# PixArt-alpha/PixArt-sigma

Hardware: AMD Instinct MI355X
Metric: denoising steps/sec (fwd+bwd) PixArt-Sigma-XL/2 1024px bs16 @1/2/4/8 GPU (higher is better)
Workload: dtype fp16; 1 GPU; PixArt-Sigma-XL/2 1024px training step (fwd+bwd+clip+AdamW), batch 16/GPU, L=300 text tokens, DP=1 RCCL all-reduce; model=PixArtMS_XL_2, global_batch=16, seq_len=4096, parallelism=dp1, grad_checkpoint=False, optimizer=adamw, text_lens=all 300

## Files before the change

### pixart_sigma_amd/csrc/attn.hip

```cpp
#include "common.h"
#include "../../include/pixart_hip.h"
#include <utility>
#include <cstdlib>

namespace {
using namespace pxa;

constexpr int DH = 72;
constexpr int NCH = DH / 8;
constexpr int KSTEPS = 5;
constexpr int ROWB = 192;
constexpr int TILE_B = 64 * ROWB;
constexpr int BKV = 64;
constexpr float RESCALE_LOG2 = 6.0f;
constexpr int NDMA = TILE_B / 1024 / 4;

struct AttnParams {
  const bf16_t *Q, *K, *V, *dO;
  bf16_t *O, *dQ, *dK, *dV;
  float* LSE;
  const float* Delta;
  float *dq_colsum, *dk_colsum, *dv_colsum;
  long colsum_stride;
  long q_bs, q_ts, k_bs, k_ts, v_bs, v_ts, o_bs, o_ts;
  int q_hs, k_hs, v_hs, o_hs;
  long dq_bs, dq_ts, dk_bs, dk_ts, dv_bs, dv_ts;
  int dq_hs, dk_hs, dv_hs;
  int B, H, Nq, Nk;
  const int* kv_start; const int* kv_len;
  float scale, scale_log2;
  float dk_scale;
  int nx;
  const bf16_t* stats;
  int Nq64;
};

#ifndef ATTN_XCD_HEADS
#define ATTN_XCD_HEADS 1
#endif
__device__ __forceinline__ void block_coords(const AttnParams& p, int& bx, int& h, int& b) {
  int v = blockIdx.x;
#if ATTN_XCD_HEADS
  const int T = gridDim.x, xq = T >> 3, xr = T & 7, xcd = v & 7;
  v = xcd * xq + min(xcd, xr) + (v >> 3);
#endif
  bx = v % p.nx;
  const int hb = v / p.nx;
  h = hb % p.H;
  b = hb / p.H;
}

__device__ __forceinline__ void kv_range(const AttnParams& p, int b, long& kbase, long& vbase, long& dkbase, long& dvbase, int& len) {
  if (p.kv_start) {
    const long s = p.kv_start[b];
    kbase = s * p.k_ts; vbase = s * p.v_ts; dkbase = s * p.dk_ts; dvbase = s * p.dv_ts; len = p.kv_len[b];
  } else {
    kbase = (long)b * p.k_bs; vbase = (long)b * p.v_bs; dkbase = (long)b * p.dk_bs; dvbase = (long)b * p.dv_bs; len = p.Nk;
  }
}


__device__ __forceinline__ int soff(int r, int c) { return r * ROWB + ((c ^ ((r >> 2) & 3)) << 4); }

__device__ __forceinline__ void tile_sync() {
  lds_dma_wait<0>();
  __syncthreads();
}
__device__ __forceinline__ void settle(bf16x8 (&f)[5]) { asm volatile("" : "+v"(f[0]), "+v"(f[1]), "+v"(f[2]), "+v"(f[3]), "+v"(f[4])); }
struct DmaPlan { int row[NDMA], coff[NDMA]; };
__device__ __forceinline__ void dma_plan(DmaPlan& pl, int wave, int lane) {
#pragma unroll
  for (int i = 0; i < NDMA; i++) {
    const int p = (i * 4 + wave) * 64 + lane, r = p / 12, cl = p - r * 12;
    const int c = cl ^ ((r >> 2) & 3);
    pl.row[i] = r;
    pl.coff[i] = c < NCH ? c * 8 : -1;
  }
}
template <bool FULL>
__device__ __forceinline__ void dma_tile(char* lds, const bf16_t* __restrict__ base, int ts, int row0, int nrows, const DmaPlan& pl, int wave) {
#pragma unroll
  for (int i = 0; i < NDMA; i++) {
    const int gr = FULL ? row0 + pl.row[i] : min(row0 + pl.row[i], nrows - 1);
    const unsigned off = (unsigned)(gr * ts + pl.coff[i]);
    if (pl.coff[i] >= 0)
      lds_dma16(base + off, lds + (i * 4 + wave) * 1024);
  }
}
#ifndef ATTN_FOLD_DELTA
#define ATTN_FOLD_DELTA 1
#endif
#define PXA_OPERAND_MINUS_ONE_X2 (((PXA_OPERAND_ONE_BITS | 0x8000u) << 16) | PXA_OPERAND_ONE_BITS | 0x8000u)
#define PXA_OPERAND_MINUS_ONE_X1 (PXA_OPERAND_ONE_BITS | 0x8000u)
__device__ __forceinline__ uint2 split3(float x) {
  const bf16_t h = (bf16_t)x;
  const float r1 = x - (float)h;
  const bf16_t m = (bf16_t)r1;
  const bf16_t l = (bf16_t)(r1 - (float)m);
  bf16x2 a, b; a[0] = h; a[1] = m; b[0] = l; b[1] = (bf16_t)0.f;
  return make_uint2(__builtin_bit_cast(uint32_t, a), __builtin_bit_cast(uint32_t, b));
}
__device__ __forceinline__ void init_pads(char* tile, int pad, int tid) {
  for (int i = tid; i < BKV * 3; i += 256) {
// ... 1551 lines not shown
    if (j + 1 >= T) break;
    body(IntC<1>{});
    kdma += j + 7 < T ? kstep : 0;  vdma += j + 5 < T ? vstep : 0;
    if (j + 2 >= T) break;
    body(IntC<2>{});
    kdma += j + 8 < T ? kstep : 0;  vdma += j + 6 < T ? vstep : 0;
    if (j + 3 >= T) break;
    body(IntC<3>{});
    kdma += j + 9 < T ? kstep : 0;  vdma += j + 7 < T ? vstep : 0;
  }
  lds_wait_all<0>(kf);
  lds_dma_wait<0>();
#if FWD4_TRACE
  if (blockIdx.x == 0 && tid == 0) { fwd4_trace_buf[0] = tr_wait; fwd4_trace_buf[1] = tr_a; fwd4_trace_buf[2] = tr_b; fwd4_trace_buf[3] = tr_n; }
#endif

  mfma_drain();
#pragma unroll
  for (int s = 0; s < QS; s++) {
    const float la = __shfl(o[s].v[4][0][0], 32 + (lane & 15)), lb = __shfl(o[s].v[4][1][0], 32 + (lane & 15));
    const float l = (lane & 16) ? lb : la;
    const float inv = l > 0.f ? 1.f / l : 0.f, invo = __shfl_xor(inv, 16);
    const int q0w = bx * 256 + wave * 64 + s * 32;
    store_rows16(p.O + (long)b * p.o_bs + (long)q0w * p.o_ts + (long)h * p.o_hs, p.o_ts, o[s], (lane & 16) ? invo : inv, (lane & 16) ? inv : invo,
                 q0w + (lane & 15) < p.Nq, q0w + 16 + (lane & 15) < p.Nq, lane);
    if (qvalid[s] && hi == 0 && p.LSE) p.LSE[((long)b * p.H + h) * p.Nq + q[s]] = mc[s] + log2f(l);
  }
}

#define PXA_WAIT_STR "s_waitcnt lgkmcnt(%3)\n\t"
template <int W = -1> __device__ __forceinline__ void mfma32_va_first(f32x16& d, const bf16x8& a, const bf16x8& b) {
  if constexpr (W >= 0) asm volatile(PXA_WAIT_STR PXA_MFMA32_ASM " %0, %1, %2, 0" : "=&v"(d) : "v"(a), "a"(b), "n"(W));
  else asm volatile(PXA_MFMA32_ASM " %0, %1, %2, 0" : "=&v"(d) : "v"(a), "a"(b));
}
template <int W = -1> __device__ __forceinline__ void mfma32_va(f32x16& d, const bf16x8& a, const bf16x8& b) {
  if constexpr (W >= 0) asm volatile(PXA_WAIT_STR PXA_MFMA32_ASM " %0, %1, %2, %0" : "+v"(d) : "v"(a), "a"(b), "n"(W));
  else asm volatile(PXA_MFMA32_ASM " %0, %1, %2, %0" : "+v"(d) : "v"(a), "a"(b));
}
template <int W = -1> __device__ __forceinline__ void mfma32_vv_first(f32x16& d, const bf16x8& a, const bf16x8& b) {
  if constexpr (W >= 0) asm volatile(PXA_WAIT_STR PXA_MFMA32_ASM " %0, %1, %2, 0" : "=&v"(d) : "v"(a), "v"(b), "n"(W));
  else asm volatile(PXA_MFMA32_ASM " %0, %1, %2, 0" : "=&v"(d) : "v"(a), "v"(b));
}
template <int W = -1> __device__ __forceinline__ void mfma32_vv(f32x16& d, const bf16x8& a, const bf16x8& b) {
  if constexpr (W >= 0) asm volatile(PXA_WAIT_STR PXA_MFMA32_ASM " %0, %1, %2, %0" : "+v"(d) : "v"(a), "v"(b), "n"(W));
  else asm volatile(PXA_MFMA32_ASM " %0, %1, %2, %0" : "+v"(d) : "v"(a), "v"(b));
}
template <int W = -1> __device__ __forceinline__ void mfma32_acc(f32x16& d, const bf16x8& a, const bf16x8& b) {
  if constexpr (W >= 0) asm volatile(PXA_WAIT_STR PXA_MFMA32_ASM " %0, %1, %2, %0" : "+a"(d) : "v"(a), "v"(b), "n"(W));
  else asm volatile(PXA_MFMA32_ASM " %0, %1, %2, %0" : "+a"(d) : "v"(a), "v"(b));
}
#ifndef PXA_ATTN_DKV4_DEFAULT
#define PXA_ATTN_DKV4_DEFAULT 1
#endif
#ifndef DKV4_ABL
#define DKV4_ABL 0
#endif
constexpr int DKV4_STAGES = 4;
constexpr int dkv4_nreads(int i) { const int k = ((i % 22) + 22) % 22; return k < 10 ? 1 : 2; }
template <bool PRE>
__global__ __launch_bounds__(256, 1) void attn_bwd_dkv4_kernel(AttnParams p) {
  __shared__ __attribute__((aligned(16))) char smem[DKV4_STAGES * STAGE_B];
  const int tid = threadIdx.x, lane = tid & 63, wave = __builtin_amdgcn_readfirstlane(tid >> 6), hi = lane >> 5;
  int bx, h, b;
  block_coords(p, bx, h, b);
  const long kbase = (long)b * p.k_bs, vbase = (long)b * p.v_bs, dkbase = (long)b * p.dk_bs, dvbase = (long)b * p.dv_bs;
  typedef unsigned u32x4 __attribute__((ext_vector_type(4)));

  const bf16_t* Qp = p.Q + (long)b * p.q_bs + (long)h * p.q_hs;
  const bf16_t* Dp = p.dO + (long)b * p.o_bs + (long)h * p.o_hs;
  const bf16_t* Ls = p.stats + ((long)b * p.H + h) * p.Nq64 * 8;
  const bf16_t* Ds = Ls + (long)p.B * p.H * p.Nq64 * 8;
  const int qts = (int)p.q_ts, ots = (int)p.o_ts;
  const int T = p.Nq / BKV;
  const float c = p.scale_log2;

  DmaPlan pl;
  dma_plan(pl, wave, lane);
  unsigned offQ[NDMA], offD[NDMA];
  unsigned long long dmask[NDMA];
#pragma unroll
  for (int i = 0; i < NDMA; i++) {
    offQ[i] = (unsigned)(pl.row[i] * qts + pl.coff[i]) * 2u;
    offD[i] = (unsigned)(pl.row[i] * ots + pl.coff[i]) * 2u;
    dmask[i] = __builtin_amdgcn_ballot_w64(pl.coff[i] >= 0);
  }
  const unsigned lds0 = (unsigned)(uintptr_t)LDS_PTR(char, smem);
  const unsigned wbase = __builtin_amdgcn_readfirstlane(wave * 1024);
  const long qstep = (long)BKV * qts, ostep = (long)BKV * ots;
  const unsigned stat_off = (unsigned)lane * 16u;
  const bf16_t* statp = (wave & 1) ? Ds : Ls;
  const unsigned stat_dst = __builtin_amdgcn_readfirstlane((wave & 1) ? 2 * TILE_B + STAT_B : TILE_B);
  const bf16_t* qnext = Qp;
  const bf16_t* dnext = Dp;
  const bf16_t* snext = statp;
  auto issue_part = [&](auto pc, unsigned sb) {
    constexpr int P = decltype(pc)::value;
    const unsigned wb = wbase + sb, so = stat_off, sd = stat_dst + sb;
    const bf16_t* sn = snext;
    if constexpr (P == 0) dma_pair<0, TILE_B + STAT_B>(dmask[0], wb, offQ[0], qnext, offD[0], dnext);
    if constexpr (P == 1) dma_pair<4096, TILE_B + STAT_B + 4096>(dmask[1], wb, offQ[1], qnext, offD[1], dnext);
    if constexpr (P == 2) dma_pair<8192, TILE_B + STAT_B + 8192>(dmask[2], wb, offQ[2], qnext, offD[2], dnext);
    if constexpr (P == 3) asm volatile("s_mov_b32 m0, %0\n\ts_nop 0\n\tglobal_load_lds_dwordx4 %1, %2" :: "s"(sd), "v"(so), "s"(sn) : "memory");
  };
  int tfetch = 0;
  auto advance = [&]() {
    const bool more = tfetch + 1 < T;
    qnext += more ? qstep : 0; dnext += more ? ostep : 0; snext += more ? (long)BKV * 8 : 0;
    tfetch++;
  };
  auto issue = [&](unsigned sb) { issue_part(IntC<0>{}, sb); issue_part(IntC<1>{}, sb); issue_part(IntC<2>{}, sb); issue_part(IntC<3>{}, sb); advance(); };

  FragAddr fa;
  frag_addr(fa, lane);
  int r4[2];
#pragma unroll
  for (int sub = 0; sub < 2; sub++) r4[sub] = hi ? TILE_B + (sub * 32 + (lane & 31)) * 16 : fa.rb[0] + 2 * 64 + sub * 32 * ROWB;
  struct Bases { unsigned r0, r1, r40, r41, t0, t1; };
  auto bases = [&](unsigned st) -> Bases { return Bases{st + (unsigned)fa.rb[0], st + (unsigned)fa.rb[1], st + (unsigned)r4[0], st + (unsigned)r4[1],
                                                        st + (unsigned)fa.tb[0], st + (unsigned)fa.tb[1]}; };
  constexpr int DOFF = TILE_B + STAT_B;

  for (int st = 0; st < DKV4_STAGES; st++) {
    init_pads(smem + st * STAGE_B, 0, tid);
    init_pads(smem + st * STAGE_B + DOFF, 0, tid);
  }
  f32x16 dk[2][3], dv[2][3];
#pragma unroll
  for (int kb = 0; kb < 2; kb++) {
    zero3(dk[kb]); zero3(dv[kb]);
#pragma unroll
    for (int dt = 0; dt < 3; dt++) { to_agpr(dk[kb][dt]); to_agpr(dv[kb][dt]); }
  }
  f32x16 S[2][2], dP[2];
  bf16x8 pb[2][2], db[2][2];
  bf16x8 f[4];

  auto rd_frag = [&](auto subc, auto ic, bf16x8& d, const Bases& cb, const Bases& nb) {
    constexpr int SUB = decltype(subc)::value, I = decltype(ic)::value;
    if constexpr (I >= 22) {
      constexpr int ks = I - 22;
      static_assert(ks < KSTEPS - 1, "look-ahead reaches the statistics fragment");
      lds_row_asm<(SUB ? 32 * ROWB : 0) + (ks >> 1) * 64>(d, (ks & 1) ? nb.r1 : nb.r0);
    } else if constexpr (I < 5) {
      constexpr int ks = I;
      if constexpr (SUB == 0) {
        if constexpr (ks < KSTEPS - 1) lds_row_asm<32 * ROWB + (ks >> 1) * 64>(d, (ks & 1) ? cb.r1 : cb.r0);
        else lds_row_asm<0>(d, cb.r41);
      } else {
        if constexpr (ks < KSTEPS - 1) lds_row_asm<(ks >> 1) * 64>(d, (ks & 1) ? nb.r1 : nb.r0);
        else lds_row_asm<0>(d, nb.r40);
      }
    } else if constexpr (I < 10) {
      constexpr int ks = I - 5;
      if constexpr (ks < KSTEPS - 1) lds_row_asm<DOFF + SUB * 32 * ROWB + (ks >> 1) * 64>(d, (ks & 1) ? cb.r1 : cb.r0);
      else lds_row_asm<DOFF>(d, SUB ? cb.r41 : cb.r40);
    } else {
      constexpr int k = (I - 10) % 6, uu = k / 3, dt = k % 3, isq = I >= 16;
      lds_tr_asm<(isq ? 0 : DOFF) + (SUB * 2 + uu) * 16 * ROWB + dt * 64>(d, cb.t0, cb.t1);
    }
  };

  issue(lds0);
  issue(lds0 + STAGE_B);
  issue(lds0 + 2 * STAGE_B);
  int kv[2];
  bf16x8 kf[2][KSTEPS], vf[2][KSTEPS];
#pragma unroll
  for (int kb = 0; kb < 2; kb++) {
    kv[kb] = bx * 256 + wave * 64 + kb * 32 + (lane & 31);
    const bool kvok = kv[kb] < p.Nk;
    load_row_frags(kf[kb], p.K + kbase + (long)kv[kb] * p.k_ts + (long)h * p.k_hs, kvok, hi);
    load_row_frags(vf[kb], p.V + vbase + (long)kv[kb] * p.v_ts + (long)h * p.v_hs, kvok, hi);
    settle(kf[kb]);
    settle(vf[kb]);
    if (hi == 1) {
      u32x4 w = __builtin_bit_cast(u32x4, kf[kb][KSTEPS - 1]);
      w[0] = PXA_OPERAND_MINUS_ONE_X2; w[1] = PXA_OPERAND_MINUS_ONE_X1;
      kf[kb][KSTEPS - 1] = __builtin_bit_cast(bf16x8, w);
      w = __builtin_bit_cast(u32x4, vf[kb][KSTEPS - 1]);
      w[0] = PXA_OPERAND_MINUS_ONE_X2; w[1] = PXA_OPERAND_MINUS_ONE_X1;
      vf[kb][KSTEPS - 1] = __builtin_bit_cast(bf16x8, w);
    }
#pragma unroll
    for (int ks = 0; ks < KSTEPS; ks++) to_agpr(vf[kb][ks]);
  }
  lds_dma_wait<14>();
  __syncthreads();
  {
    const Bases cb = bases(lds0);
    static_for<5>([&](auto kc) {
      constexpr int ks = decltype(kc)::value;
      if constexpr (ks < KSTEPS - 1) lds_row_asm<(ks >> 1) * 64>(f[ks & 3], (ks & 1) ? cb.r1 : cb.r0);
      else lds_row_asm<0>(f[0], cb.r40);
      if constexpr (ks == 3) { lds_wait<0>(f[0]); }
      if constexpr (ks == 3) { mfma32_vv_first(S[0][0], f[0], kf[0][0]); mfma32_vv_first(S[0][1], f[0], kf[1][0]); }
    });
    asm volatile("s_waitcnt lgkmcnt(0)" : "+v"(f[0]), "+v"(f[1]), "+v"(f[2]), "+v"(f[3]));
    mfma32_vv(S[0][0], f[1], kf[0][1]); mfma32_vv(S[0][1], f[1], kf[1][1]);
    mfma32_vv(S[0][0], f[2], kf[0][2]); mfma32_vv(S[0][1], f[2], kf[1][2]);
    mfma32_vv(S[0][0], f[3], kf[0][3]); mfma32_vv(S[0][1], f[3], kf[1][3]);
    mfma32_vv(S[0][0], f[0], kf[0][4]); mfma32_vv(S[0][1], f[0], kf[1][4]);
    mfma_drain();
#pragma unroll
    for (int kb = 0; kb < 2; kb++)
#pragma unroll
      for (int g = 0; g < 16; g++) if (!PRE) S[0][kb][g] *= c;
    static_for<4>([&](auto ic) { rd_frag(IntC<0>{}, ic, f[decltype(ic)::value], cb, cb); });
  }

  int t = 0;
  auto step = [&](auto subc, const Bases& cb, const Bases& nb, unsigned fst) {
    constexpr int SUB = decltype(subc)::value, CUR = SUB, NXT = SUB ^ 1;
    auto pack_p = [&](auto gc) {
      constexpr int g0 = decltype(gc)::value;
      if constexpr (g0 >= 0 && g0 < 20) {
        constexpr int p0 = (32 * g0) / 20, p1 = (32 * (g0 + 1)) / 20;
        static_for<p1 - p0>([&](auto ec) {
          constexpr int e = p0 + decltype(ec)::value, kb = e >> 4, g = e & 15;
          if constexpr (g & 1) {
            unsigned w = (DKV4_ABL & 2) ? __builtin_bit_cast(unsigned, S[CUR][kb][g]) : pack_bf16x2(S[CUR][kb][g - 1], S[CUR][kb][g]);
            asm volatile("" : "+v"(w));
            u32x4 ww = __builtin_bit_cast(u32x4, pb[kb][g >> 3]);
            ww[(g & 7) >> 1] = w;
            pb[kb][g >> 3] = __builtin_bit_cast(bf16x8, ww);
          }
        });
      }
    };
    auto pack_ds = [&](auto gc) {
      constexpr int g0 = decltype(gc)::value;
      if constexpr (g0 >= 20 && g0 < 32) {
        constexpr int p0 = (32 * (g0 - 20)) / 12, p1 = (32 * (g0 - 19)) / 12;
        static_for<p1 - p0>([&](auto ec) {
          constexpr int e = p0 + decltype(ec)::value, kb = e >> 4, g = e & 15;
          if constexpr (g & 1) {
            unsigned w = (DKV4_ABL & 2) ? __builtin_bit_cast(unsigned, dP[kb][g]) : pack_bf16x2(dP[kb][g - 1], dP[kb][g]);
            asm volatile("" : "+v"(w));
            u32x4 ww = __builtin_bit_cast(u32x4, db[kb][g >> 3]);
            ww[(g & 7) >> 1] = w;
            db[kb][g >> 3] = __builtin_bit_cast(bf16x8, ww);
          }
        });
      }
    };
    auto valu = [&](auto gic) {
      constexpr int gi = decltype(gic)::value;
      pack_p(IntC<gi - 2>{});
      pack_ds(IntC<gi - 2>{});
      if constexpr (gi < 20) {
        constexpr int e0 = (32 * gi) / 20, e1 = (32 * (gi + 1)) / 20;
        static_for<e1 - e0>([&](auto ec) {
          constexpr int e = e0 + decltype(ec)::value;
          if (!(DKV4_ABL & 1)) S[CUR][e >> 4][e & 15] = __builtin_amdgcn_exp2f(S[CUR][e >> 4][e & 15]);
          asm volatile("" : "+v"(S[CUR][e >> 4][e & 15]));
        });
      } else if constexpr (gi < 32) {
        constexpr int e0 = (32 * (gi - 20)) / 12, e1 = (32 * (gi - 19)) / 12;
        static_for<e1 - e0>([&](auto ec) {
          constexpr int e = e0 + decltype(ec)::value;
          if (!(DKV4_ABL & 4)) dP[e >> 4][e & 15] *= S[CUR][e >> 4][e & 15];
          asm volatile("" : "+v"(dP[e >> 4][e & 15]));
        });
      } else {
        constexpr int e0 = (32 * (gi - 32)) / 12, e1 = (32 * (gi - 31)) / 12;
        static_for<e1 - e0>([&](auto ec) {
          constexpr int e = e0 + decltype(ec)::value;
          if (!PRE && !(DKV4_ABL & 4)) S[NXT][e >> 4][e & 15] *= c;
          asm volatile("" : "+v"(S[NXT][e >> 4][e & 15]));
        });
      }
    };
    auto mma = [&](auto ic, auto kbc, auto wc) {
      constexpr int i = decltype(ic)::value, kb = decltype(kbc)::value, W = decltype(wc)::value, q = (i + 2 * SUB) & 3;
      if constexpr (DKV4_ABL & 32) { if constexpr (W >= 0) lds_wait<(W >= 0 ? W : 0)>(f[q]); return; }
      if constexpr (i < 5) { if constexpr (i == 0) mfma32_vv_first<W>(S[NXT][kb], f[q], kf[kb][0]); else mfma32_vv<W>(S[NXT][kb], f[q], kf[kb][i]); }
      else if constexpr (i < 10) { if constexpr (i == 5) mfma32_va_first<W>(dP[kb], f[q], vf[kb][0]); else mfma32_va<W>(dP[kb], f[q], vf[kb][i - 5]); }
      else if constexpr (i < 16) mfma32_acc<W>(dv[kb][(i - 10) % 3], f[q], pb[kb][(i - 10) / 3]);
      else mfma32_acc<W>(dk[kb][(i - 16) % 3], f[q], db[kb][(i - 16) / 3]);
    };
    static_for<11>([&](auto kc) {
      constexpr int i = 2 * decltype(kc)::value;
      if constexpr (SUB == 0 && i == 18) {
        lds_dma_wait<7>();
        __syncthreads();
        if constexpr (!(DKV4_ABL & 16)) issue_part(IntC<0>{}, fst);
      }
      if constexpr (SUB == 0 && i == 20 && !(DKV4_ABL & 16)) issue_part(IntC<1>{}, fst);
      if constexpr (SUB == 1 && i == 0 && !(DKV4_ABL & 16)) issue_part(IntC<2>{}, fst);
      if constexpr (SUB == 1 && i == 2 && !(DKV4_ABL & 16)) { issue_part(IntC<3>{}, fst); advance(); }
      mma(IntC<i>{}, IntC<0>{}, IntC<dkv4_nreads(i + 2) + dkv4_nreads(i + 3)>{});
      __builtin_amdgcn_sched_barrier(0);
      valu(IntC<2 * i>{});
      __builtin_amdgcn_sched_barrier(0);
      mma(IntC<i>{}, IntC<1>{}, IntC<-1>{});
      __builtin_amdgcn_sched_barrier(0);
      if constexpr (!(DKV4_ABL & 8)) rd_frag(subc, IntC<i + 4>{}, f[(i + 2 * SUB) & 3], cb, nb);
      valu(IntC<2 * i + 1>{});
      __builtin_amdgcn_sched_barrier(0);
      mma(IntC<i + 1>{}, IntC<0>{}, IntC<-1>{});
      __builtin_amdgcn_sched_barrier(0);
      valu(IntC<2 * i + 2>{});
      __builtin_amdgcn_sched_barrier(0);
      mma(IntC<i + 1>{}, IntC<1>{}, IntC<-1>{});
      __builtin_amdgcn_sched_barrier(0);
      if constexpr (!(DKV4_ABL & 8)) rd_frag(subc, IntC<i + 5>{}, f[(i + 1 + 2 * SUB) & 3], cb, nb);
      valu(IntC<2 * i + 3>{});
      __builtin_amdgcn_sched_barrier(0);
    });
  };
  unsigned cur = lds0, nx = lds0 + STAGE_B, fst = lds0 + 3 * STAGE_B;
  Bases cb = bases(cur);
  for (t = 0; t < T; t++) {
    const Bases nb = bases(nx);
    step(IntC<0>{}, cb, nb, fst);
    step(IntC<1>{}, cb, nb, fst);
    cb = nb;
    fst = cur;
    cur = nx;
    nx = nx + STAGE_B == lds0 + DKV4_STAGES * STAGE_B ? lds0 : nx + STAGE_B;
  }
  asm volatile("s_waitcnt lgkmcnt(0)" : "+v"(f[0]), "+v"(f[1]), "+v"(f[2]), "+v"(f[3]));
  lds_dma_wait<0>();
  mfma_drain();
#pragma unroll
  for (int kb = 0; kb < 2; kb++) {
    const bool kvok = kv[kb] < p.Nk;
    if (kvok) {
      store_rows(p.dK + dkbase + (long)kv[kb] * p.dk_ts + (long)h * p.dk_hs, dk[kb], p.dk_scale, hi);
      store_rows(p.dV + dvbase + (long)kv[kb] * p.dv_ts + (long)h * p.dv_hs, dv[kb], 1.f, hi);
    }
    if (p.dk_colsum) colsum_rows(p.dk_colsum + (b % PXA_COLSUM_SLOTS) * p.colsum_stride + h * DH, dk[kb], p.dk_scale, kvok, hi, lane);
    if (p.dv_colsum) colsum_rows(p.dv_colsum + (b % PXA_COLSUM_SLOTS) * p.colsum_stride + h * DH, dv[kb], 1.f, kvok, hi, lane);
  }
}



#ifndef PXA_ATTN_DQ4_DEFAULT
#define PXA_ATTN_DQ4_DEFAULT 1
#endif
constexpr int DQ4_STAGES = 5;
#ifndef DQ4_FOLD_LSE
#define DQ4_FOLD_LSE 1
#endif
template <bool PRE_>
__global__ __launch_bounds__(256, 1) void attn_bwd_dq4_kernel(AttnParams p) {
  constexpr bool PRE = PRE_ && DQ4_FOLD_LSE;
  constexpr int STG = 2 * TILE_B;
  __shared__ __attribute__((aligned(16))) char smem[DQ4_STAGES * STG];
  const int tid = threadIdx.x, lane = tid & 63, wave = __builtin_amdgcn_readfirstlane(tid >> 6), hi = lane >> 5;
  int bx, h, b;
  block_coords(p, bx, h, b);
  const bf16_t* Kp = p.K + (long)b * p.k_bs + (long)h * p.k_hs;
  const bf16_t* Vp = p.V + (long)b * p.v_bs + (long)h * p.v_hs;
  const int kts = (int)p.k_ts, vts = (int)p.v_ts;
  const int T = p.Nk / BKV;
  const float c = p.scale_log2;
  typedef unsigned u32x4 __attribute__((ext_vector_type(4)));

  DmaPlan pl;
  dma_plan(pl, wave, lane);
  unsigned offK[NDMA], offV[NDMA];
  unsigned long long dmask[NDMA];
#pragma unroll
  for (int i = 0; i < NDMA; i++) {
    offK[i] = (unsigned)(pl.row[i] * kts + pl.coff[i]) * 2u;
    offV[i] = (unsigned)(pl.row[i] * vts + pl.coff[i]) * 2u;
    dmask[i] = __builtin_amdgcn_ballot_w64(pl.coff[i] >= 0);
  }
  const unsigned lds0 = (unsigned)(uintptr_t)LDS_PTR(char, smem);
  const unsigned wbase = __builtin_amdgcn_readfirstlane(wave * 1024);
  const long kstep = (long)BKV * kts, vstep = (long)BKV * vts;
  const bf16_t* knext = Kp;
  const bf16_t* vnext = Vp;
  int tfetch = 0;
  auto issue_part = [&](auto pc, unsigned sb) {
    constexpr int P = decltype(pc)::value;
    dma_pair<P * 4096, TILE_B + P * 4096>(dmask[P], wbase + sb, offK[P], knext, offV[P], vnext);
  };
  auto advance = [&]() {
    const bool more = tfetch + 1 < T;
    knext += more ? kstep : 0; vnext += more ? vstep : 0;
    tfetch++;
  };
  auto issue = [&](unsigned sb) { issue_part(IntC<0>{}, sb); issue_part(IntC<1>{}, sb); issue_part(IntC<2>{}, sb); advance(); };
// ... 200 lines not shown
    cb = nb;
    cur = nx;
    nx = nx + STG == ring_end ? lds0 : nx + STG;
    fst = fst + STG == ring_end ? lds0 : fst + STG;
  }
  {
    asm volatile("s_waitcnt lgkmcnt(0)" : "+v"(fs[0][0]), "+v"(fs[0][1]), "+v"(fs[0][2]), "+v"(fs[0][3]), "+v"(fs[0][4]));
    static_for<5>([&](auto tc) { rd_ktr(IntC<1>{}, tc, fs[1][decltype(tc)::value], pbs); });
    wait_set(fs[1]);
    static_for<20>([&](auto gc) {
      constexpr int g = decltype(gc)::value, tt = g >> 2, qb = (g >> 1) & 1, half = g & 1;
      mfma16_acc(dq[qb].v[tt][half], fs[1][tt], __builtin_bit_cast(bf16x8, half ? dyu[1][qb] : dxu[1][qb]));
    });
  }
  lds_dma_wait<0>();
  mfma_drain();
#pragma unroll
  for (int qb = 0; qb < 2; qb++) {
    const int q0w = bx * 256 + wave * 64 + qb * 32;
    const bool ok0 = q0w + (lane & 15) < p.Nq, ok1 = q0w + 16 + (lane & 15) < p.Nq;
    store_rows16(p.dQ + (long)b * p.dq_bs + (long)q0w * p.dq_ts + (long)h * p.dq_hs, p.dq_ts, dq[qb], p.scale, p.scale, ok0, ok1, lane);
    if (p.dq_colsum) colsum_rows16(p.dq_colsum + (b % PXA_COLSUM_SLOTS) * p.colsum_stride + h * DH, dq[qb], p.scale, ok0, ok1, lane);
  }
}

enum class AttnFwd { kvres, fwd4, fwd2, fwd1 };
enum class AttnPre { none, rows, strided };
enum class AttnDq { kvres, dq4, dq2, r2 };
enum class AttnDkv { dkv4, dkv2, dkv2_plain, dkv5, dkv3, r2 };

int fwd_grid(AttnFwd k, AttnParams& p, int& qpb) {
  if (k == AttnFwd::kvres) {
    qpb = p.Nq >= 4096 ? 4096 : (p.Nq + 511) / 512 * 512;
    p.nx = (p.Nq + qpb - 1) / qpb;
    return 0;
  }
  p.nx = k == AttnFwd::fwd1 ? (p.Nq + 127) / 128 : (p.Nq + 255) / 256;
  PXA_CHECK((long)p.nx * p.H * p.B < (1L << 31), "pxa_attn_fwd: grid too large");
  return 0;
}

int dq_grid(AttnDq k, AttnParams& p, int& qpb) {
  if (k == AttnDq::kvres) {
    qpb = p.Nq >= 4096 ? 4096 : (p.Nq + 255) / 256 * 256;
    p.nx = (p.Nq + qpb - 1) / qpb;
    return 0;
  }
  p.nx = (p.Nq + 127) / 128;
  PXA_CHECK((long)p.nx * p.H * p.B < (1L << 31), "pxa_attn_bwd: grid too large");
  if (k == AttnDq::dq4) p.nx = (p.Nq + 255) / 256;
  return 0;
}

int dkv_grid(AttnDkv k, AttnParams& p, int max_k) {
  const bool keys128 = k == AttnDkv::dkv2 || k == AttnDkv::dkv2_plain || k == AttnDkv::r2;
  p.nx = keys128 ? (max_k + 127) / 128 : (max_k + 255) / 256;
  PXA_CHECK((long)p.nx * p.H * p.B < (1L << 31), "pxa_attn_bwd: grid too large");
  return 0;
}

bool fwd_kvres_available() { return lds_optin(reinterpret_cast<const void*>(attn_fwd_kvres_kernel), KVRES_TILES * 2 * TILE_B) == hipSuccess; }

int launch_fwd(AttnFwd k, AttnParams p, int max_k, hipStream_t stream) {
  int qpb = 0;
  if (int rc = fwd_grid(k, p, qpb)) return rc;
  if (k == AttnFwd::kvres) {
    const int tiles = (max_k + BKV - 1) / BKV, lds = tiles * 2 * TILE_B;
    hipLaunchKernelGGL(attn_fwd_kvres_kernel, dim3(p.nx * p.H * p.B), dim3(512), lds, stream, p, qpb, tiles);
    PXA_LAUNCH_CHECK();
    return 0;
  }
  const dim3 grid(p.nx * p.H * p.B), block(256);
  if (k == AttnFwd::fwd4) hipLaunchKernelGGL(attn_fwd4_kernel, grid, block, 0, stream, p);
  else if (k == AttnFwd::fwd2) hipLaunchKernelGGL(attn_fwd2_kernel, grid, block, 0, stream, p);
  else hipLaunchKernelGGL(attn_fwd_kernel, grid, block, 0, stream, p);
  PXA_LAUNCH_CHECK();
  return 0;
}

bool dq_kvres_available() { return lds_optin(reinterpret_cast<const void*>(attn_bwd_dq_kvres_kernel), KVRES_TILES * 2 * TILE_B) == hipSuccess; }

int launch_prepass(AttnPre k, const AttnParams& p, float* delta, bf16_t* stats, float inv_c, hipStream_t stream) {
  if (stats && p.Nq64 != p.Nq) {
    const int n = p.B * p.H * (p.Nq64 - p.Nq);
    hipLaunchKernelGGL(attn_stats_pad_kernel, dim3((n + 255) / 256), dim3(256), 0, stream, stats, p.B * p.H, p.Nq, p.Nq64);
  }
  if (k == AttnPre::rows) {
    const long tokens = (long)p.B * p.Nq;
    hipLaunchKernelGGL(attn_delta_rows_kernel, dim3((tokens + DELTA_TOK - 1) / DELTA_TOK), dim3(256), 0, stream, p.O, p.dO, delta, p.H, p.Nq, tokens,
                       p.LSE, stats, p.Nq64, inv_c);
  } else if (k == AttnPre::strided) {
    const long total = (long)p.B * p.Nq * p.H;
    hipLaunchKernelGGL(attn_delta_kernel, dim3((total + 255) / 256), dim3(256), 0, stream, p.O, p.dO, delta,
                       p.o_bs, p.o_ts, p.o_hs, p.o_bs, p.o_ts, p.o_hs, p.B, p.H, p.Nq, p.LSE, stats, p.Nq64, inv_c);
  }
  PXA_LAUNCH_CHECK();
  return 0;
}

int launch_dq(AttnDq k, bool prescaled, AttnParams p, int max_k, float* delta, bf16_t* stats, float inv_c, hipStream_t stream) {
  int qpb = 0;
  if (int rc = dq_grid(k, p, qpb)) return rc;
  if (k == AttnDq::kvres) {
    const int tiles = (max_k + BKV - 1) / BKV, lds = tiles * 2 * TILE_B;
    hipLaunchKernelGGL(attn_bwd_dq_kvres_kernel, dim3(p.nx * p.H * p.B), dim3(512), lds, stream, p, qpb, tiles, delta, stats, inv_c);
    PXA_LAUNCH_CHECK();
    return 0;
  }
  if (k == AttnDq::dq4) {
    if (prescaled) hipLaunchKernelGGL(attn_bwd_dq4_kernel<true>, dim3(p.nx * p.H * p.B), dim3(256), 0, stream, p);
    else hipLaunchKernelGGL(attn_bwd_dq4_kernel<false>, dim3(p.nx * p.H * p.B), dim3(256), 0, stream, p);
  } else hipLaunchKernelGGL(attn_bwd_dq2_kernel, dim3(p.nx * p.H * p.B), dim3(256), 0, stream, p);
  PXA_LAUNCH_CHECK();
  return 0;
}

int launch_dkv(AttnDkv k, bool prescaled, AttnParams p, int max_k, hipStream_t stream) {
  if (int rc = dkv_grid(k, p, max_k)) return rc;
  if (p.nx > 0) {
    const dim3 grid(p.nx * p.H * p.B), block(256);
    if (k == AttnDkv::dkv4 && prescaled) hipLaunchKernelGGL(attn_bwd_dkv4_kernel<true>, grid, block, 0, stream, p);
    else if (k == AttnDkv::dkv4) hipLaunchKernelGGL(attn_bwd_dkv4_kernel<false>, grid, block, 0, stream, p);
    else if (k == AttnDkv::dkv2) hipLaunchKernelGGL(attn_bwd_dkv2_kernel<1>, grid, block, 0, stream, p);
    else hipLaunchKernelGGL(attn_bwd_dkv2_kernel<0>, grid, block, 0, stream, p);
  }
  PXA_LAUNCH_CHECK();
  return 0;
}
}

#include "attn_ab.h"

namespace {
int fill(AttnParams& p, const pxa_attn_args* a) {
  PXA_CHECK(a, "attn: null args");
  PXA_CHECK(a->head_dim == DH, "attn: head_dim %d unsupported (PixArt XL/2 uses 72)", a->head_dim);
  PXA_CHECK(a->B > 0 && a->H > 0 && a->Nq > 0 && a->Nk >= 0, "attn: bad shape");
  PXA_CHECK(!a->kv_start == !a->kv_len, "attn: kv_start/kv_len must both be given");
  p.Q = (const bf16_t*)a->q; p.K = (const bf16_t*)a->k; p.V = (const bf16_t*)a->v; p.dO = (const bf16_t*)a->d_o;
  p.O = (bf16_t*)a->o; p.dQ = (bf16_t*)a->dq; p.dK = (bf16_t*)a->dk; p.dV = (bf16_t*)a->dv;
  p.LSE = a->lse; p.Delta = a->delta;
  p.dq_colsum = a->dq_colsum; p.dk_colsum = a->dk_colsum; p.dv_colsum = a->dv_colsum; p.colsum_stride = a->colsum_stride;
  p.q_bs = a->q_bs; p.q_ts = a->q_ts; p.q_hs = a->q_hs;
  p.k_bs = a->k_bs; p.k_ts = a->k_ts; p.k_hs = a->k_hs;
  p.v_bs = a->v_bs; p.v_ts = a->v_ts; p.v_hs = a->v_hs;
  p.o_bs = a->o_bs; p.o_ts = a->o_ts; p.o_hs = a->o_hs;
  p.dq_bs = a->dq_bs; p.dq_ts = a->dq_ts; p.dq_hs = a->dq_hs;
  p.dk_bs = a->dk_bs; p.dk_ts = a->dk_ts; p.dk_hs = a->dk_hs;
  p.dv_bs = a->dv_bs; p.dv_ts = a->dv_ts; p.dv_hs = a->dv_hs;
  p.B = a->B; p.H = a->H; p.Nq = a->Nq; p.Nk = a->Nk;
  p.kv_start = a->kv_start; p.kv_len = a->kv_len;
  p.scale = a->scale; p.scale_log2 = a->scale * 1.4426950408889634f; p.dk_scale = a->scale;
  if (a->q_prescaled) { p.scale_log2 = 1.0f; p.dk_scale = 0.6931471805599453f; }
  p.stats = (const bf16_t*)a->bwd_stats; p.Nq64 = (a->Nq + BKV - 1) / BKV * BKV;
  const long strides[] = {p.q_ts, p.k_ts, p.v_ts, p.o_ts, p.q_hs, p.k_hs, p.v_hs, p.o_hs, p.q_bs, p.k_bs, p.v_bs, p.o_bs};
  for (long s : strides) PXA_CHECK(s % 8 == 0, "attn: strides must be multiples of 8 elements (16-byte rows)");
  return 0;
}

struct Knobs {
  bool fwd1;
  bool no_kvres;
  const char* fwd4;
  const char* dkv;
  const char* dq;
  bool no_prepass;
};
Knobs read_knobs(bool backward) {
  static const bool fwd1 = getenv("PXA_ATTN_FWD1") != nullptr;
  static const bool no_kvres = getenv("PXA_ATTN_NO_KVRES") != nullptr;
  Knobs k{fwd1, no_kvres, nullptr, nullptr, nullptr, false};
  if (backward) {
    k.dkv = getenv("PXA_ATTN_DKV");
    k.dq = getenv("PXA_ATTN_DQ");
    k.no_prepass = getenv("PXA_ATTN_BWD_NO_PREPASS") != nullptr;
  } else {
    k.fwd4 = getenv("PXA_ATTN_FWD4");
  }
  return k;
}

bool keys_fit_lds(const AttnParams& p, int max_k) { return max_k > 0 && max_k <= KVRES_TILES * BKV && p.Nq >= 512; }

AttnFwd choose_fwd(const AttnParams& p, int max_k, const Knobs& k) {
  if (!k.no_kvres && !k.fwd1 && keys_fit_lds(p, max_k) && fwd_kvres_available()) return AttnFwd::kvres;
  const bool two = !k.fwd1 && p.Nq >= 256;
  const bool f4_ok = two && !p.kv_start && p.Nk >= BKV && p.Nk % BKV == 0;
  if (f4_ok && (k.fwd4 ? atoi(k.fwd4) != 0 : (PXA_ATTN_FWD4_DEFAULT && p.Nk >= 8 * BKV))) return AttnFwd::fwd4;
  return two ? AttnFwd::fwd2 : AttnFwd::fwd1;
}

bool choose_dq_kvres(const AttnParams& p, int max_k, const Knobs& k) {
  return !k.no_kvres && ATTN_FOLD_DELTA && p.dQ && keys_fit_lds(p, max_k) && dq_kvres_available();
}

AttnPre choose_prepass(const AttnParams& p, const Knobs& k, bool dq_kvres) {
  if (k.no_prepass || dq_kvres) return AttnPre::none;
  const bool token_rows = p.o_hs == DH && p.o_ts == (long)p.H * DH && p.o_bs == (long)p.Nq * p.o_ts && p.H <= 16 && ((uintptr_t)p.O % 16) == 0 && ((uintptr_t)p.dO % 16) == 0;
  return token_rows ? AttnPre::rows : AttnPre::strided;
}

AttnDq choose_dq(const AttnParams& p, const Knobs& k) {
  int mode = ATTN_FOLD_DELTA ? (k.dq ? atoi(k.dq) : PXA_ATTN_DQ_DEFAULT) : 0;
  const bool dq4_ok = ATTN_FOLD_DELTA && !p.kv_start && p.Nk % BKV == 0 && p.Nk >= 2 * BKV && p.Nq >= 256;
  if (mode == 4 && !dq4_ok) mode = 1;
  if (!k.dq && mode == 1 && PXA_ATTN_DQ4_DEFAULT && dq4_ok) mode = 4;
  return mode == 4 ? AttnDq::dq4 : mode ? AttnDq::dq2 : AttnDq::r2;
}

AttnDkv choose_dkv(const AttnParams& p, const Knobs& k) {
  int mode = k.dkv ? atoi(k.dkv) : PXA_ATTN_DKV_DEFAULT;
  if (!p.stats || !p.dK) mode = 0;
  const bool dkv4_ok = p.stats && !p.kv_start && p.Nk % BKV == 0 && p.Nk >= 256 && p.Nq % BKV == 0 && p.Nq >= 2 * BKV;
  if (mode >= 4 && !dkv4_ok) mode = 2;
  if (!k.dkv && mode == 2 && PXA_ATTN_DKV4_DEFAULT && dkv4_ok) mode = 4;
  switch (mode) {
    case 5: return AttnDkv::dkv5;
    case 4: return AttnDkv::dkv4;
    case 3: return AttnDkv::dkv3;
    case 2: return AttnDkv::dkv2;
    case 1: return AttnDkv::dkv2_plain;
    default: return AttnDkv::r2;
  }
}
}

namespace {
struct AttnPlan {
  int max_k;
  AttnFwd fwd;
  AttnPre pre;
  AttnDq dq;
  AttnDkv dkv;
  bf16_t* stats;
};

int plan_fwd(const pxa_attn_args* a, AttnParams& p, AttnPlan& g) {
  if (int rc = fill(p, a)) return rc;
  PXA_CHECK(p.Q && p.K && p.V && p.O, "pxa_attn_fwd: null tensor");
  const Knobs k = read_knobs(false);
  g.max_k = a->max_kv_len > 0 ? a->max_kv_len : p.Nk;
  g.fwd = choose_fwd(p, g.max_k, k);
  return 0;
}

int plan_bwd(const pxa_attn_args* a, AttnParams& p, AttnPlan& g) {
  if (int rc = fill(p, a)) return rc;
  PXA_CHECK(p.Q && p.K && p.V && p.O && p.dO && p.LSE && a->delta, "pxa_attn_bwd: null tensor");
  PXA_CHECK((p.dQ || p.dK) && (!p.dK == !p.dV), "pxa_attn_bwd: need dq and/or both of dk, dv (a NULL gradient skips the kernel that produces it)");
  for (long s : {p.dq_ts, p.dk_ts, p.dv_ts, (long)p.dq_hs, (long)p.dk_hs, (long)p.dv_hs, p.dq_bs, p.dk_bs, p.dv_bs})
    PXA_CHECK(s % 4 == 0, "pxa_attn_bwd: gradient strides must be multiples of 4 elements");
  const Knobs k = read_knobs(true);
  g.max_k = a->max_kv_len > 0 ? a->max_kv_len : p.Nk;
  g.dkv = choose_dkv(p, k);
  const bool dq_kvres = choose_dq_kvres(p, g.max_k, k);
  g.stats = g.dkv != AttnDkv::r2 ? (bf16_t*)a->bwd_stats : nullptr;
  g.pre = choose_prepass(p, k, dq_kvres);
  g.dq = dq_kvres ? AttnDq::kvres : choose_dq(p, k);
  return 0;
}
}

extern "C" int pxa_attn_fwd(const pxa_attn_args* a, hipStream_t stream) {
  AttnParams p; AttnPlan g;
  if (int rc = plan_fwd(a, p, g)) return rc;
  return launch_fwd(g.fwd, p, g.max_k, stream);
}

extern "C" long pxa_attn_bwd_stats_bytes(int B, int H, int Nq) { return 2L * B * H * ((Nq + BKV - 1) / BKV * BKV) * 16; }

extern "C" int pxa_attn_bwd(const pxa_attn_args* a, hipStream_t stream) {
  AttnParams p; AttnPlan g;
  if (int rc = plan_bwd(a, p, g)) return rc;
  const bool pre = a->q_prescaled != 0;
  const float inv_c = 1.0f / p.scale_log2;

  if (int rc = launch_prepass(g.pre, p, a->delta, g.stats, inv_c, stream)) return rc;
  if (p.dQ) {
    const int rc = g.dq == AttnDq::r2 ? launch_dq_ab(p, stream) : launch_dq(g.dq, pre, p, g.max_k, a->delta, g.stats, inv_c, stream);
    if (rc) return rc;
  }
  if (p.dK) {
    switch (g.dkv) {
      case AttnDkv::dkv4: case AttnDkv::dkv2: case AttnDkv::dkv2_plain: return launch_dkv(g.dkv, pre, p, g.max_k, stream);
      case AttnDkv::dkv5: case AttnDkv::dkv3: case AttnDkv::r2: return launch_dkv_ab(g.dkv, pre, p, g.max_k, stream);
    }
  }
  return 0;
}

extern "C" int pxa_attn_plan(const pxa_attn_args* a, int backward, char* out, int out_len) {
  AttnParams p; AttnPlan g;
  int n, qpb = 0;
  if (!backward) {
    if (int rc = plan_fwd(a, p, g)) return rc;
    if (int rc = fwd_grid(g.fwd, p, qpb)) return rc;
    PXA_CHECK(out && out_len > 0, "pxa_attn_plan: no text buffer");
    static const char* const name[] = {"kvres", "fwd4", "fwd2", "fwd1"};
    static const char* const kernel[] = {"attn_fwd_kvres_kernel", "attn_fwd4_kernel", "attn_fwd2_kernel", "attn_fwd_kernel"};
    n = snprintf(out, out_len, "fwd=%s fwd_kernel=%s fwd_nx=%d", name[(int)g.fwd], kernel[(int)g.fwd], p.nx);
  } else {
    if (int rc = plan_bwd(a, p, g)) return rc;
    const bool pre = a->q_prescaled != 0;
    static const char* const pre_name[] = {"none", "rows", "strided"};
    static const char* const pre_kernel[] = {"-", "attn_delta_rows_kernel", "attn_delta_kernel"};
    static const char* const dq_name[] = {"kvres", "dq4", "dq2", "r2"};
    static const char* const dq_kernel[] = {"attn_bwd_dq_kvres_kernel", "attn_bwd_dq4_kernel", "attn_bwd_dq2_kernel", "attn_bwd_dq_kernel"};
    static const char* const dkv_name[] = {"dkv4", "dkv2", "dkv2_plain", "dkv5", "dkv3", "r2"};
    static const char* const dkv_kernel[] = {"attn_bwd_dkv4_kernel", "attn_bwd_dkv2_kernel<1>", "attn_bwd_dkv2_kernel<0>", "attn_bwd_dkv5_kernel", "attn_bwd_dkv3_kernel<2>",
                                             "attn_bwd_dkv_kernel"};
    int dq_nx = 0, dkv_nx = 0;
    if (p.dQ) {
      if (int rc = dq_grid(g.dq, p, qpb)) return rc;
      dq_nx = p.nx;
    }
    if (p.dK) {
      if (int rc = dkv_grid(g.dkv, p, g.max_k)) return rc;
      dkv_nx = p.nx;
    }
    PXA_CHECK(out && out_len > 0, "pxa_attn_plan: no text buffer");
    const bool dq_pre = p.dQ && g.dq == AttnDq::dq4, dkv_pre = p.dK && (g.dkv == AttnDkv::dkv4 || g.dkv == AttnDkv::dkv5);
    n = snprintf(out, out_len, "pre=%s dq=%s dkv=%s pre_kernel=%s dq_kernel=%s%s dq_nx=%d dkv_kernel=%s%s dkv_nx=%d", pre_name[(int)g.pre],
                 p.dQ ? dq_name[(int)g.dq] : "skip", p.dK ? dkv_name[(int)g.dkv] : "skip", pre_kernel[(int)g.pre],
                 p.dQ ? dq_kernel[(int)g.dq] : "-", dq_pre ? (pre ? "<true>" : "<false>") : "", dq_nx,
                 p.dK ? dkv_kernel[(int)g.dkv] : "-", dkv_pre ? (pre ? "<true>" : "<false>") : "", dkv_nx);
  }
  PXA_CHECK(n < out_len, "pxa_attn_plan: text buffer of %d bytes is too small", out_len);
  return 0;
}

#if FWD4_TRACE
extern "C" int pxa_attn_fwd4_trace(unsigned long long* out) { return hipMemcpyFromSymbol(out, HIP_SYMBOL(fwd4_trace_buf), sizeof(fwd4_trace_buf)) == hipSuccess ? 0 : -1; }
#endif
```

Before: 2.456 steps/s.

## Make dK/dV attention backward kernel persistent with cross-item prefetch

Adds a persistent variant of the dkv4 backward kernel that launches one block per CU (rounded to a multiple of 8) and loops over (key-block, head, batch) items. At the end of each item's Q loop, the DMA pipeline already wraps into the next item's Q/dO/stats tiles, and the next K/V fragments are requested before the current dK/dV rows are stored. This is meant to hide per-block prologue and epilogue latency and the tail effect. It adds loop bookkeeping and register pressure, and it relies on items being at least the CU count. Enabled by default and controllable through an env knob.

```diff
diff --git a/pixart_sigma_amd/csrc/attn.hip b/pixart_sigma_amd/csrc/attn.hip
--- a/pixart_sigma_amd/csrc/attn.hip
+++ b/pixart_sigma_amd/csrc/attn.hip
@@ -33,15 +33,15 @@
   int nx;
   const bf16_t* stats;
   int Nq64;
+  int items;
 };
 
 #ifndef ATTN_XCD_HEADS
 #define ATTN_XCD_HEADS 1
 #endif
-__device__ __forceinline__ void block_coords(const AttnParams& p, int& bx, int& h, int& b) {
-  int v = blockIdx.x;
+__device__ __forceinline__ void item_coords(const AttnParams& p, int v, int total, int& bx, int& h, int& b) {
 #if ATTN_XCD_HEADS
-  const int T = gridDim.x, xq = T >> 3, xr = T & 7, xcd = v & 7;
+  const int xq = total >> 3, xr = total & 7, xcd = v & 7;
   v = xcd * xq + min(xcd, xr) + (v >> 3);
 #endif
   bx = v % p.nx;
@@ -49,6 +49,7 @@
   h = hb % p.H;
   b = hb / p.H;
 }
+__device__ __forceinline__ void block_coords(const AttnParams& p, int& bx, int& h, int& b) { item_coords(p, blockIdx.x, gridDim.x, bx, h, b); }
 
 __device__ __forceinline__ void kv_range(const AttnParams& p, int b, long& kbase, long& vbase, long& dkbase, long& dvbase, int& len) {
   if (p.kv_start) {
@@ -1706,24 +1707,32 @@
 #ifndef PXA_ATTN_DKV4_DEFAULT
 #define PXA_ATTN_DKV4_DEFAULT 1
 #endif
+#ifndef PXA_ATTN_DKV4_PERSIST_DEFAULT
+#define PXA_ATTN_DKV4_PERSIST_DEFAULT 1
+#endif
 #ifndef DKV4_ABL
 #define DKV4_ABL 0
 #endif
 constexpr int DKV4_STAGES = 4;
 constexpr int dkv4_nreads(int i) { const int k = ((i % 22) + 22) % 22; return k < 10 ? 1 : 2; }
-template <bool PRE>
+template <bool PRE, bool PERS = false>
 __global__ __launch_bounds__(256, 1) void attn_bwd_dkv4_kernel(AttnParams p) {
   __shared__ __attribute__((aligned(16))) char smem[DKV4_STAGES * STAGE_B];
   const int tid = threadIdx.x, lane = tid & 63, wave = __builtin_amdgcn_readfirstlane(tid >> 6), hi = lane >> 5;
+  const int total = PERS ? p.items : (int)gridDim.x;
+  int item = blockIdx.x;
   int bx, h, b;
-  block_coords(p, bx, h, b);
-  const long kbase = (long)b * p.k_bs, vbase = (long)b * p.v_bs, dkbase = (long)b * p.dk_bs, dvbase = (long)b * p.dv_bs;
+  item_coords(p, item, total, bx, h, b);
   typedef unsigned u32x4 __attribute__((ext_vector_type(4)));
 
-  const bf16_t* Qp = p.Q + (long)b * p.q_bs + (long)h * p.q_hs;
-  const bf16_t* Dp = p.dO + (long)b * p.o_bs + (long)h * p.o_hs;
-  const bf16_t* Ls = p.stats + ((long)b * p.H + h) * p.Nq64 * 8;
-  const bf16_t* Ds = Ls + (long)p.B * p.H * p.Nq64 * 8;
+  const long stats_half = (long)p.B * p.H * p.Nq64 * 8;
+  auto head_rows = [&](int b_, int h_, const bf16_t*& q, const bf16_t*& d, const bf16_t*& s) {
+    q = p.Q + (long)b_ * p.q_bs + (long)h_ * p.q_hs;
+    d = p.dO + (long)b_ * p.o_bs + (long)h_ * p.o_hs;
+    s = p.stats + ((long)b_ * p.H + h_) * p.Nq64 * 8 + ((wave & 1) ? stats_half : 0);
+  };
+  const bf16_t *Qp, *Dp, *statp;
+  head_rows(b, h, Qp, Dp, statp);
   const int qts = (int)p.q_ts, ots = (int)p.o_ts;
   const int T = p.Nq / BKV;
   const float c = p.scale_log2;
@@ -1742,7 +1751,6 @@
   const unsigned wbase = __builtin_amdgcn_readfirstlane(wave * 1024);
   const long qstep = (long)BKV * qts, ostep = (long)BKV * ots;
   const unsigned stat_off = (unsigned)lane * 16u;
-  const bf16_t* statp = (wave & 1) ? Ds : Ls;
   const unsigned stat_dst = __builtin_amdgcn_readfirstlane((wave & 1) ? 2 * TILE_B + STAT_B : TILE_B);
   const bf16_t* qnext = Qp;
   const bf16_t* dnext = Dp;
@@ -1757,11 +1765,33 @@
     if constexpr (P == 3) asm volatile("s_mov_b32 m0, %0\n\ts_nop 0\n\tglobal_load_lds_dwordx4 %1, %2" :: "s"(sd), "v"(so), "s"(sn) : "memory");
   };
   int tfetch = 0;
+  const bf16_t *nq = nullptr, *nd = nullptr, *ns = nullptr;
+  long qs = qstep, os = ostep, ss = (long)BKV * 8;
+  bool nlast = true;
+  auto set_next = [&]() {
+    nlast = item + (int)gridDim.x >= total;
+    if (!nlast) {
+      int nbx, nh, nb_;
+      item_coords(p, item + (int)gridDim.x, total, nbx, nh, nb_);
+      head_rows(nb_, nh, nq, nd, ns);
+    } else {
+      nq = Qp + (long)(T - 1) * qstep; nd = Dp + (long)(T - 1) * ostep; ns = statp + (long)(T - 1) * BKV * 8;
+    }
+  };
   auto advance = [&]() {
-    const bool more = tfetch + 1 < T;
-    qnext += more ? qstep : 0; dnext += more ? ostep : 0; snext += more ? (long)BKV * 8 : 0;
-    tfetch++;
-  };
+    if constexpr (PERS) {
+      const bool wrap = ++tfetch == T;
+      qnext = wrap ? nq : qnext + qs; dnext = wrap ? nd : dnext + os; snext = wrap ? ns : snext + ss;
+      const long keep = (wrap & nlast) ? 0L : -1L;
+      qs &= keep; os &= keep; ss &= keep;
+      tfetch = wrap ? 0 : tfetch;
+    } else {
+      const bool more = tfetch + 1 < T;
+      qnext += more ? qstep : 0; dnext += more ? ostep : 0; snext += more ? (long)BKV * 8 : 0;
+      tfetch++;
+    }
+  };
+  if constexpr (PERS) set_next();
   auto issue = [&](unsigned sb) { issue_part(IntC<0>{}, sb); issue_part(IntC<1>{}, sb); issue_part(IntC<2>{}, sb); issue_part(IntC<3>{}, sb); advance(); };
 
   FragAddr fa;
@@ -1779,12 +1809,15 @@
     init_pads(smem + st * STAGE_B + DOFF, 0, tid);
   }
   f32x16 dk[2][3], dv[2][3];
+  auto zero_acc = [&]() {
 #pragma unroll
   for (int kb = 0; kb < 2; kb++) {
     zero3(dk[kb]); zero3(dv[kb]);
 #pragma unroll
     for (int dt = 0; dt < 3; dt++) { to_agpr(dk[kb][dt]); to_agpr(dv[kb][dt]); }
   }
+  };
+  zero_acc();
   f32x16 S[2][2], dP[2];
   bf16x8 pb[2][2], db[2][2];
   bf16x8 f[4];
@@ -1819,12 +1852,18 @@
   issue(lds0 + 2 * STAGE_B);
   int kv[2];
   bf16x8 kf[2][KSTEPS], vf[2][KSTEPS];
+  auto request_kv = [&]() {
 #pragma unroll
   for (int kb = 0; kb < 2; kb++) {
     kv[kb] = bx * 256 + wave * 64 + kb * 32 + (lane & 31);
     const bool kvok = kv[kb] < p.Nk;
-    load_row_frags(kf[kb], p.K + kbase + (long)kv[kb] * p.k_ts + (long)h * p.k_hs, kvok, hi);
-    load_row_frags(vf[kb], p.V + vbase + (long)kv[kb] * p.v_ts + (long)h * p.v_hs, kvok, hi);
+    load_row_frags(kf[kb], p.K + (long)b * p.k_bs + (long)kv[kb] * p.k_ts + (long)h * p.k_hs, kvok, hi);
+    load_row_frags(vf[kb], p.V + (long)b * p.v_bs + (long)kv[kb] * p.v_ts + (long)h * p.v_hs, kvok, hi);
+  }
+  };
+  auto settle_kv = [&]() {
+#pragma unroll
+  for (int kb = 0; kb < 2; kb++) {
     settle(kf[kb]);
     settle(vf[kb]);
     if (hi == 1) {
@@ -1838,10 +1877,12 @@
 #pragma unroll
     for (int ks = 0; ks < KSTEPS; ks++) to_agpr(vf[kb][ks]);
   }
+  };
+  request_kv();
+  settle_kv();
   lds_dma_wait<14>();
   __syncthreads();
-  {
-    const Bases cb = bases(lds0);
+  auto first_block = [&](const Bases& cb) {
     static_for<5>([&](auto kc) {
       constexpr int ks = decltype(kc)::value;
       if constexpr (ks < KSTEPS - 1) lds_row_asm<(ks >> 1) * 64>(f[ks & 3], (ks & 1) ? cb.r1 : cb.r0);
@@ -1860,7 +1901,7 @@
 #pragma unroll
       for (int g = 0; g < 16; g++) if (!PRE) S[0][kb][g] *= c;
     static_for<4>([&](auto ic) { rd_frag(IntC<0>{}, ic, f[decltype(ic)::value], cb, cb); });
-  }
+  };
 
   int t = 0;
   auto step = [&](auto subc, const Bases& cb, const Bases& nb, unsigned fst) {
@@ -1964,27 +2005,42 @@
   };
   unsigned cur = lds0, nx = lds0 + STAGE_B, fst = lds0 + 3 * STAGE_B;
   Bases cb = bases(cur);
-  for (t = 0; t < T; t++) {
-    const Bases nb = bases(nx);
-    step(IntC<0>{}, cb, nb, fst);
-    step(IntC<1>{}, cb, nb, fst);
-    cb = nb;
-    fst = cur;
-    cur = nx;
-    nx = nx + STAGE_B == lds0 + DKV4_STAGES * STAGE_B ? lds0 : nx + STAGE_B;
-  }
-  asm volatile("s_waitcnt lgkmcnt(0)" : "+v"(f[0]), "+v"(f[1]), "+v"(f[2]), "+v"(f[3]));
-  lds_dma_wait<0>();
-  mfma_drain();
-#pragma unroll
-  for (int kb = 0; kb < 2; kb++) {
-    const bool kvok = kv[kb] < p.Nk;
-    if (kvok) {
-      store_rows(p.dK + dkbase + (long)kv[kb] * p.dk_ts + (long)h * p.dk_hs, dk[kb], p.dk_scale, hi);
-      store_rows(p.dV + dvbase + (long)kv[kb] * p.dv_ts + (long)h * p.dv_hs, dv[kb], 1.f, hi);
-    }
-    if (p.dk_colsum) colsum_rows(p.dk_colsum + (b % PXA_COLSUM_SLOTS) * p.colsum_stride + h * DH, dk[kb], p.dk_scale, kvok, hi, lane);
-    if (p.dv_colsum) colsum_rows(p.dv_colsum + (b % PXA_COLSUM_SLOTS) * p.colsum_stride + h * DH, dv[kb], 1.f, kvok, hi, lane);
+  for (;;) {
+    first_block(cb);
+    for (t = 0; t < T; t++) {
+      const Bases nb = bases(nx);
+      step(IntC<0>{}, cb, nb, fst);
+      step(IntC<1>{}, cb, nb, fst);
+      cb = nb;
+      fst = cur;
+      cur = nx;
+      nx = nx + STAGE_B == lds0 + DKV4_STAGES * STAGE_B ? lds0 : nx + STAGE_B;
+    }
+    asm volatile("s_waitcnt lgkmcnt(0)" : "+v"(f[0]), "+v"(f[1]), "+v"(f[2]), "+v"(f[3]));
+    const bool more = PERS && item + (int)gridDim.x < total;
+    if (!more) lds_dma_wait<0>();
+    mfma_drain();
+    const int eh = h, eb = b, ekv[2] = {kv[0], kv[1]};
+    if (more) {
+      item += (int)gridDim.x;
+      item_coords(p, item, total, bx, h, b);
+      request_kv();
+    }
+#pragma unroll
+    for (int kb = 0; kb < 2; kb++) {
+      const bool kvok = ekv[kb] < p.Nk;
+      if (kvok) {
+        store_rows(p.dK + (long)eb * p.dk_bs + (long)ekv[kb] * p.dk_ts + (long)eh * p.dk_hs, dk[kb], p.dk_scale, hi);
+        store_rows(p.dV + (long)eb * p.dv_bs + (long)ekv[kb] * p.dv_ts + (long)eh * p.dv_hs, dv[kb], 1.f, hi);
+      }
+      if (p.dk_colsum) colsum_rows(p.dk_colsum + (eb % PXA_COLSUM_SLOTS) * p.colsum_stride + eh * DH, dk[kb], p.dk_scale, kvok, hi, lane);
+      if (p.dv_colsum) colsum_rows(p.dv_colsum + (eb % PXA_COLSUM_SLOTS) * p.colsum_stride + eh * DH, dv[kb], 1.f, kvok, hi, lane);
+    }
+    if (!more) break;
+    head_rows(b, h, Qp, Dp, statp);
+    set_next();
+    settle_kv();
+    zero_acc();
   }
 }
 
@@ -2291,6 +2347,25 @@
   return 0;
 }
 
+int attn_cu_count() {
+  static int cus[64] = {};
+  int dev = 0;
+  if (hipGetDevice(&dev) != hipSuccess || dev < 0 || dev >= 64) return 0;
+  if (!cus[dev]) {
+    hipDeviceProp_t prop;
+    if (hipGetDeviceProperties(&prop, dev) == hipSuccess) cus[dev] = prop.multiProcessorCount;
+  }
+  return cus[dev];
+}
+
+int persistent_grid(const AttnParams& p, int tiles, int min_tiles) {
+  const long items = (long)p.nx * p.H * p.B;
+  const int g = attn_cu_count() & ~7;
+  return g >= 8 && items >= g && tiles >= min_tiles ? g : 0;
+}
+constexpr int DKV4_PERS_MIN_TILES = 4;
+int dkv4_persistent_grid(const AttnParams& p, bool want) { return want ? persistent_grid(p, p.Nq / BKV, DKV4_PERS_MIN_TILES) : 0; }
+
 int dkv_grid(AttnDkv k, AttnParams& p, int max_k) {
   const bool keys128 = k == AttnDkv::dkv2 || k == AttnDkv::dkv2_plain || k == AttnDkv::r2;
   p.nx = keys128 ? (max_k + 127) / 128 : (max_k + 255) / 256;
@@ -2354,12 +2429,16 @@
   return 0;
 }
 
-int launch_dkv(AttnDkv k, bool prescaled, AttnParams p, int max_k, hipStream_t stream) {
+int launch_dkv(AttnDkv k, bool prescaled, bool persistent, AttnParams p, int max_k, hipStream_t stream) {
   if (int rc = dkv_grid(k, p, max_k)) return rc;
   if (p.nx > 0) {
     const dim3 grid(p.nx * p.H * p.B), block(256);
-    if (k == AttnDkv::dkv4 && prescaled) hipLaunchKernelGGL(attn_bwd_dkv4_kernel<true>, grid, block, 0, stream, p);
-    else if (k == AttnDkv::dkv4) hipLaunchKernelGGL(attn_bwd_dkv4_kernel<false>, grid, block, 0, stream, p);
+    p.items = (int)grid.x;
+    const int pg = k == AttnDkv::dkv4 ? dkv4_persistent_grid(p, persistent) : 0;
+    if (k == AttnDkv::dkv4 && !pg && prescaled) hipLaunchKernelGGL(attn_bwd_dkv4_kernel<true>, grid, block, 0, stream, p);
+    else if (k == AttnDkv::dkv4 && !pg) hipLaunchKernelGGL(attn_bwd_dkv4_kernel<false>, grid, block, 0, stream, p);
+    else if (k == AttnDkv::dkv4 && prescaled) hipLaunchKernelGGL((attn_bwd_dkv4_kernel<true, true>), dim3(pg), block, 0, stream, p);
+    else if (k == AttnDkv::dkv4) hipLaunchKernelGGL((attn_bwd_dkv4_kernel<false, true>), dim3(pg), block, 0, stream, p);
     else if (k == AttnDkv::dkv2) hipLaunchKernelGGL(attn_bwd_dkv2_kernel<1>, grid, block, 0, stream, p);
     else hipLaunchKernelGGL(attn_bwd_dkv2_kernel<0>, grid, block, 0, stream, p);
   }
@@ -2404,6 +2483,7 @@
   const char* dkv;
   const char* dq;
   bool no_prepass;
+  const char* dkv4_persist;
 };
 Knobs read_knobs(bool backward) {
   static const bool fwd1 = getenv("PXA_ATTN_FWD1") != nullptr;
@@ -2413,6 +2493,7 @@
     k.dkv = getenv("PXA_ATTN_DKV");
     k.dq = getenv("PXA_ATTN_DQ");
     k.no_prepass = getenv("PXA_ATTN_BWD_NO_PREPASS") != nullptr;
+    k.dkv4_persist = getenv("PXA_ATTN_DKV4_PERSIST");
   } else {
     k.fwd4 = getenv("PXA_ATTN_FWD4");
   }
@@ -2471,6 +2552,8 @@
   AttnPre pre;
   AttnDq dq;
   AttnDkv dkv;
+  bool dkv_persist;
+  bool dkv_persist_knob;
   bf16_t* stats;
 };
 
@@ -2492,6 +2575,8 @@
   const Knobs k = read_knobs(true);
   g.max_k = a->max_kv_len > 0 ? a->max_kv_len : p.Nk;
   g.dkv = choose_dkv(p, k);
+  g.dkv_persist_knob = k.dkv4_persist && atoi(k.dkv4_persist) != 0;
+  g.dkv_persist = k.dkv4_persist ? g.dkv_persist_knob : PXA_ATTN_DKV4_PERSIST_DEFAULT != 0;
   const bool dq_kvres = choose_dq_kvres(p, g.max_k, k);
   g.stats = g.dkv != AttnDkv::r2 ? (bf16_t*)a->bwd_stats : nullptr;
   g.pre = choose_prepass(p, k, dq_kvres);
@@ -2521,7 +2606,7 @@
   }
   if (p.dK) {
     switch (g.dkv) {
-      case AttnDkv::dkv4: case AttnDkv::dkv2: case AttnDkv::dkv2_plain: return launch_dkv(g.dkv, pre, p, g.max_k, stream);
+      case AttnDkv::dkv4: case AttnDkv::dkv2: case AttnDkv::dkv2_plain: return launch_dkv(g.dkv, pre, g.dkv_persist, p, g.max_k, stream);
       case AttnDkv::dkv5: case AttnDkv::dkv3: case AttnDkv::r2: return launch_dkv_ab(g.dkv, pre, p, g.max_k, stream);
     }
   }
@@ -2559,10 +2644,11 @@
     }
     PXA_CHECK(out && out_len > 0, "pxa_attn_plan: no text buffer");
     const bool dq_pre = p.dQ && g.dq == AttnDq::dq4, dkv_pre = p.dK && (g.dkv == AttnDkv::dkv4 || g.dkv == AttnDkv::dkv5);
+    const bool dkv_pers = p.dK && g.dkv == AttnDkv::dkv4 && g.dkv_persist_knob && dkv4_persistent_grid(p, true) > 0;
     n = snprintf(out, out_len, "pre=%s dq=%s dkv=%s pre_kernel=%s dq_kernel=%s%s dq_nx=%d dkv_kernel=%s%s dkv_nx=%d", pre_name[(int)g.pre],
                  p.dQ ? dq_name[(int)g.dq] : "skip", p.dK ? dkv_name[(int)g.dkv] : "skip", pre_kernel[(int)g.pre],
                  p.dQ ? dq_kernel[(int)g.dq] : "-", dq_pre ? (pre ? "<true>" : "<false>") : "", dq_nx,
-                 p.dK ? dkv_kernel[(int)g.dkv] : "-", dkv_pre ? (pre ? "<true>" : "<false>") : "", dkv_nx);
+                 p.dK ? dkv_kernel[(int)g.dkv] : "-", dkv_pers ? (pre ? "<true,true>" : "<false,true>") : dkv_pre ? (pre ? "<true>" : "<false>") : "", dkv_nx);
   }
   PXA_CHECK(n < out_len, "pxa_attn_plan: text buffer of %d bytes is too small", out_len);
   return 0;
```

After: 2.441 steps/s. No clear change (-0.6%).
